# xuhao1/TaichiSLAM

Measured on AMD Instinct MI355X. Metric: depth-frames/s integrated (640x480->512^3 TSDF), higher is better.
Workload: dtype f16 storage / f32 + int64 fixed-point arithmetic; 1 GPU; BASELINE configs[1]: single 640x480 u16 depth stream (sphere room r=3 m, 1 deg/frame) -> DenseTSDF 512^3 / 2 cm, recast_step 2, max_ray 5 m; one stream+submap per GPU

## Files before the change

taichislam_amd/csrc/tsl_integrate.hip:

```cpp
#include "tsl_tsdf.hpp"
#include <hip/hip_ext.h>

namespace tsl {

#ifdef TSL_TIMING
#define TSL_T0() const int _wv = (blockIdx.x * (int)blockDim.x + (int)threadIdx.x) >> 6
#define TSL_TICK(F, k) do { long long _n = wall_clock64(); if (lane_id() == 0 && _wv < 16384) (F).dbg[_wv * 16 + (k)] = _n; } while (0)
#else
#define TSL_T0() do {} while (0)
#define TSL_TICK(F, k) do {} while (0)
#endif

#define SCATTER_TILE 4096

struct RayRegs { float pf0, pf1, pf2, d0, d1, d2, P0, P1, P2, w; long long qden; int n; };

__device__ __forceinline__ uint32_t wave_min_u32(uint32_t v)
{
    for (int d = 32; d > 0; d >>= 1) { const uint32_t o = (uint32_t)__shfl_xor((int)v, d); v = o < v ? o : v; }
    return v;
}
__device__ __forceinline__ RayRegs make_ray(const uint4 rec, int n, const FrameParams& P)
{
    RayRegs R;
// ... 553 lines not shown
{
    if (all_small) {
#pragma unroll
        for (int q = 0; q < N; ++q) nv[q] = apply_update_f(old[q], from_fix32(qn[q]), from_fix32(qd[q]));
    } else {
#pragma unroll
        for (int q = 0; q < N; ++q) nv[q] = apply_update_f(old[q], from_fix(qn[q]), from_fix(qd[q]));
    }
}

__device__ __forceinline__ int uni(int v) { return __builtin_amdgcn_readfirstlane(v); }
#define IT_UNIT 0
#define IT_POOL 1
#define IT_SLAB 2
#define IT_NP   3
#define IT_TMALL 4
#define IT_FMASK 5
#define IT_OFF  6
#define IT_N    (IT_OFF + TSL_NB)
#define IT_WORDS (IT_N + TSL_NB + 2)
#define NRANGE (PLAN_NCLS * (TSL_NB + 1))

template <bool TEX, bool FASTDIV, int NT, int SPT, int WPE>
__global__ void __launch_bounds__(NT, WPE) k_integrate_batch(MapDev M, BatchDev B, int kind)
{
    constexpr int CSEGS = SPT * NT, VPT = TSL_BRK3 / NT, CH = VPT < FLUSH_CHUNK ? VPT : FLUSH_CHUNK;
    static_assert(VPT <= 16, "the written / first-touch masks hold 16 voxels per thread");
#ifdef TSL_EXP_SLOT16
    __shared__ ulonglong2 s_acc[TSL_BRK3];
#define S_NUM(i) s_acc[i].x
#define S_DEN(i) s_acc[i].y
#else
    __shared__ unsigned long long s_num[TSL_BRK3];
    __shared__ unsigned long long s_den[TSL_BRK3];
#define S_NUM(i) s_num[i]
#define S_DEN(i) s_den[i]
#endif
    __shared__ unsigned long long s_keys[CSEGS];
    __shared__ uint32_t s_win[TEX ? TSL_BRK3 : 1];
    __shared__ int s_bin[64];
    __shared__ int s_claim[2];
    __shared__ int s_uq[TSL_NB];
    __shared__ int s_cum[NRANGE + 1];
    __shared__ int s_it[3][IT_WORDS];
    uint32_t okmask = 0u;
#pragma unroll
    for (int q = 0; q < TSL_NB; ++q) if (q < B.n) {
        const FrameDev& Fq = B.f[q];
// ... 51 lines not shown
            int pool = e.z;
            if (fm == 0u) { fm = 1u; pool = -1; }
            it[IT_UNIT] = kq < 0 ? 1 : 0; it[IT_POOL] = pool; it[IT_SLAB] = kq < 0 ? 0 : e.w; it[IT_NP] = kq < 0 ? 1 : (e.y >> 16) & ((1 << PART_NP_BITS) - 1);
            it[IT_TMALL] = (int)tm; it[IT_FMASK] = (int)fm;
        }
    };
    const int r0 = uni(s_claim[0]);
    if (r0 >= total) return;
    { int kq, io, in; const int4 e = entry_of(r0, &kq); info_of(e, kq, &io, &in); commit(0, e, kq, io, in); }
    __syncthreads();
    auto steps_of = [&](int sl, uint32_t fm) -> int {
        int n = 0;
#pragma unroll
        for (int q = 0; q < TSL_NB; ++q) if ((fm >> q) & 1u) n += max(1, (uni(s_it[sl][IT_N + q]) + CSEGS - 1) / CSEGS);
        return n;
    };
    long long uniq = 0;
    int t = 0, slot = 0, c = 0; (void)t;
    int n_known = 0;
    bool exhausted = false;
    int f = __builtin_ctz((uint32_t)uni(s_it[0][IT_FMASK]));

    unsigned long long kk[SPT]; uint4 recs[SPT]; uint32_t wids[SPT];
#define TSL_SORT_DEAL(KIN, NSEG, FD)                                                                                    \
    {                                                                                                                   \
        int rr[SPT];                                                                                                    \
        _Pragma("unroll") for (int q = 0; q < SPT; ++q) {                                                               \
            const int i = q * NT + (int)threadIdx.x; rr[q] = -1;                                                        \
            if (i < (NSEG)) rr[q] = atomicAdd(&s_bin[63 - (int)(KIN[q] & 63ull)], 1);                                   \
        }                                                                                                               \
        __syncthreads();                                                                                                \
        if (threadIdx.x < 64) {                                                                                         \
            const int cb = s_bin[threadIdx.x]; int inc = cb;                                                            \
            for (int d = 1; d < 64; d <<= 1) { const int o = __shfl_up(inc, d); if ((int)threadIdx.x >= d) inc += o; }  \
            s_bin[threadIdx.x] = inc - cb;                                                                              \
        }                                                                                                               \
        __syncthreads();                                                                                                \
        _Pragma("unroll") for (int q = 0; q < SPT; ++q) if (rr[q] >= 0) s_keys[s_bin[63 - (int)(KIN[q] & 63ull)] + rr[q]] = KIN[q]; \
        __syncthreads();                                                                                                \
        _Pragma("unroll") for (int q = 0; q < SPT; ++q) {                                                               \
            const int i = q * NT + ((q & 1) ? NT - 1 - (int)threadIdx.x : (int)threadIdx.x);                            \
            if (i < (NSEG)) {                                                                                           \
                kk[q] = s_keys[i];                                                                                      \
                const int r = (int)((kk[q] >> (SEG_CNT_BITS + SEG_J_BITS)) & ((1u << STG_RAY_BITS) - 1));               \
                recs[q] = (FD).rayA[r];                                                                                 \
                wids[q] = TEX ? (FD).rayFirst[r] + 1u : 0u;                                                             \
            }                                                                                                           \
        }                                                                                                               \
        if (threadIdx.x < 64) s_bin[threadIdx.x] = 0;               \
    }
#define TSL_PRIME(SL, FQ)                                                                                               \
    {                                                                                                                   \
        const FrameDev& F0 = B.f[FQ];                                                                                   \
        const int off0 = uni(s_it[SL][IT_OFF + (FQ)]), nseg0 = min(uni(s_it[SL][IT_N + (FQ)]), CSEGS);                  \
        unsigned long long k0[SPT];                                                                                     \
        _Pragma("unroll") for (int q = 0; q < SPT; ++q) { const int i = q * NT + threadIdx.x; k0[q] = i < nseg0 ? F0.seg_sorted[off0 + i] : 0ull; } \
        TSL_SORT_DEAL(k0, nseg0, F0)                                                                                    \
    }

    {
#ifdef TSL_EXP_SLOT16
        for (int i = threadIdx.x; i < TSL_BRK3; i += NT) s_acc[i] = make_ulonglong2(0ull, 0ull);
#else
        ulonglong2* zn = reinterpret_cast<ulonglong2*>(s_num); ulonglong2* zd = reinterpret_cast<ulonglong2*>(s_den);
        for (int i = threadIdx.x; i < TSL_BRK3 / 2; i += NT) { zn[i] = make_ulonglong2(0ull, 0ull); zd[i] = make_ulonglong2(0ull, 0ull); }
#endif
        if (TEX) for (int i = threadIdx.x; i < TSL_BRK3; i += NT) s_win[i] = 0u;
        if (threadIdx.x < 64) s_bin[threadIdx.x] = 0;
        __syncthreads();
        TSL_PRIME(0, f)
    }
    uint32_t old[VPT];
    uint32_t vmask = 0u;
    bool have_old = false;
    for (;;) {
        const int* const it = s_it[slot];
        const int slot1 = slot == 2 ? 0 : slot + 1, slot2 = slot == 0 ? 2 : slot - 1;
        const bool unit = uni(it[IT_UNIT]) != 0;
        const int p = uni(it[IT_POOL]), rk = uni(it[IT_SLAB]);
        const uint32_t fmask = (uint32_t)uni(it[IT_FMASK]);
        const int n_f = uni(it[IT_N + f]);
        const FrameDev& F = B.f[f];
        const FrameParams& P = *B.p[f];
        const StepK K = { P.vs, P.rvs, P.T[0], P.T[1], P.T[2], M.hN, M.hNz };
        const uint32_t later = fmask >> (f + 1);
        const bool first_frame = (fmask & ((1u << f) - 1u)) == 0u, last_frame = later == 0u;
        const bool first_step = first_frame && c == 0;
        const int nseg = min(CSEGS, n_f - c * CSEGS);
        const bool last_chunk = (c + 1) * CSEGS >= n_f;
        const bool last_step = last_chunk && last_frame;
        int known = max(1, (n_f + CSEGS - 1) / CSEGS) - 1 - c + steps_of(slot, later << (f + 1));
        if (n_known >= 1) known += steps_of(slot1, (uint32_t)uni(s_it[slot1][IT_FMASK]));
        const bool do_claim = !exhausted && n_known < 2 && known <= 1;
        if (do_claim && threadIdx.x == 0) s_claim[0] = __hip_atomic_fetch_add(claim, 1, __ATOMIC_RELAXED, __HIP_MEMORY_SCOPE_AGENT);
#ifdef TSL_TIMING
        long long* const _rec = F.dbg + 131072 + (size_t)blockIdx.x * 128 + (size_t)(t < 16 ? t : 15) * 8;
        if (threadIdx.x == 0 && first_step) { _rec[0] = wall_clock64(); _rec[1] = (unit ? 1 : 0) | (uni(it[IT_NP]) << 8) | ((long long)fmask << 32); _rec[2] = 0; _rec[5] = 0; }
        if (threadIdx.x == 0 && c == 0) _rec[2] += n_f;
        long long* const _ph = F.dbg + 196608 + (size_t)blockIdx.x * 128 + (size_t)(t < 16 ? t : 15) * 8;
        if (threadIdx.x == 0 && first_step) { _ph[0] = _ph[1] = _ph[2] = _ph[3] = _ph[4] = 0; }
        const long long _ta = wall_clock64();
#endif
        const bool has_next = !last_step || n_known >= 1;
        int fx = f, cx = c + 1, slotx = slot;
        if (last_chunk) {
            cx = 0;
            if (!last_frame) fx = f + 1 + __builtin_ctz(later);
            else if (has_next) { slotx = slot1; fx = __builtin_ctz((uint32_t)uni(s_it[slotx][IT_FMASK])); }
        }
        const FrameDev& Fx = B.f[fx];
        unsigned long long kn[SPT];
        const int offx = uni(s_it[slotx][IT_OFF + fx]) + cx * CSEGS;
        const int nsegn = has_next ? min(CSEGS, uni(s_it[slotx][IT_N + fx]) - cx * CSEGS) : 0;
#pragma unroll
        for (int q = 0; q < SPT; ++q) { const int i = q * NT + threadIdx.x; kn[q] = i < nsegn ? Fx.seg_sorted[offx + i] : 0ull; }
        const uint32_t* const twr = M.tw + (size_t)(p >= 0 ? p : 0) * TSL_BRK3;
        if (first_step) { have_old = false; vmask = 0u; }
        if (!TEX && unit && p >= 0 && first_step) {
#pragma unroll
            for (int q = 0; q < VPT; ++q) old[q] = twr[q * NT + threadIdx.x];
            have_old = true;
        }
#pragma unroll
        for (int q = 0; q < SPT; ++q) {
            const int i = q * NT + ((q & 1) ? NT - 1 - (int)threadIdx.x : (int)threadIdx.x);
            if (i >= nseg) continue;
            const unsigned long long key = kk[q];
            const int cnt = (int)(key & ((1u << SEG_CNT_BITS) - 1)), j0 = (int)((key >> SEG_CNT_BITS) & ((1u << SEG_J_BITS) - 1));
            const RayRegs R = make_ray(recs[q], 0, P);
            const uint32_t wid = wids[q];
#ifndef TSL_EXP_STAGGER
#define TSL_EXP_STAGGER 27
#endif
            int off = ((int)((threadIdx.x * (unsigned)TSL_EXP_STAGGER) & 63u) * cnt) >> 6;
            for (int s = 0; s < cnt; s += 2) {
                const int ja = j0 + off; off = (off + 1 == cnt) ? 0 : off + 1;
                const int jb = j0 + off; off = (off + 1 == cnt) ? 0 : off + 1;
                int la, lb; float qa, qb;
                step_eval<FASTDIV>(R, K, ja, &la, &qa);
                step_eval<FASTDIV>(R, K, jb, &lb, &qb);
                long long na = (long long)(int)qa, nb = (long long)(int)qb;
                if (__builtin_expect(__any(!(fabsf(qa) < 2147483648.0f) || !(fabsf(qb) < 2147483648.0f)), 0)) { na = __float2ll_rn(qa); nb = __float2ll_rn(qb); }
                atomicAdd(&S_NUM(la), (unsigned long long)na);
                atomicAdd(&S_DEN(la), (unsigned long long)R.qden);
                if (TEX) atomicMax(&s_win[la], wid);
                const bool vb = s + 1 < cnt;
#ifdef TSL_EXP_ADDZERO
                atomicAdd(&S_NUM(lb), (unsigned long long)(vb ? nb : 0ll));
                atomicAdd(&S_DEN(lb), (unsigned long long)(vb ? R.qden : 0ll));
                if (TEX) atomicMax(&s_win[lb], vb ? wid : 0u);
#else
                if (vb) { atomicAdd(&S_NUM(lb), (unsigned long long)nb); atomicAdd(&S_DEN(lb), (unsigned long long)R.qden); if (TEX) atomicMax(&s_win[lb], wid); }
#endif
            }
        }
        __syncthreads();
#ifdef TSL_TIMING
        if (threadIdx.x == 0 && last_step) _rec[3] = wall_clock64();
        const long long _tb = wall_clock64();
#endif
        bool fetching = false;
        int4 ne = make_int4(0, 0, -1, 0); int nkq = 0, nio = 0, nin = 0;
        if (do_claim) {
            const int r = uni(s_claim[0]);
            if (r < total) { fetching = true; ne = entry_of(r, &nkq); } else exhausted = true;
        }
        if (has_next) TSL_SORT_DEAL(kn, nsegn, Fx)
        if (fetching) info_of(ne, nkq, &nio, &nin);
#ifdef TSL_TIMING
        const long long _tc = wall_clock64();
        if (threadIdx.x == 0) { _ph[0] += _tb - _ta; _ph[1] += _tc - _tb; _ph[4] += 1; }
#endif
        if (!last_chunk) {
            if (fetching) { commit(n_known == 0 ? slot1 : slot2, ne, nkq, nio, nin); ++n_known; __syncthreads(); }
            ++c; continue;
        }
        if (p >= 0 && threadIdx.x == 0) M.touch[p] = 1;
        if (p >= 0 && unit) {
            uint32_t* tw = M.tw + (size_t)p * TSL_BRK3;
            if (!have_old) {
#pragma unroll
                for (int q = 0; q < VPT; ++q) old[q] = tw[q * NT + threadIdx.x];
                have_old = true;
            }
            if (first_frame) {
#pragma unroll
                for (int q = 0; q < VPT; ++q) vmask |= ((old[q] >> 16) == 0u ? 1u : 0u) << (16 + q);
            }
#pragma unroll
            for (int h = 0; h < VPT; h += CH) {
                long long qn[CH], qd[CH]; uint32_t nv[CH]; bool small = true, anyu = false;
#pragma unroll
                for (int q = 0; q < CH; ++q) {
                    const int ls = acc_swz5((h + q) * NT + threadIdx.x);
// ... 35 lines not shown
                S_NUM(ls) = 0ull; S_DEN(ls) = 0ull;
                if (TEX) { F.accw[(size_t)rk * TSL_BRK3 + l] = s_win[ls]; s_win[ls] = 0u; }
            }
        } else {
#ifdef TSL_EXP_SLOT16
            for (int i = threadIdx.x; i < TSL_BRK3; i += NT) s_acc[i] = make_ulonglong2(0ull, 0ull);
#else
            ulonglong2* zn = reinterpret_cast<ulonglong2*>(s_num); ulonglong2* zd = reinterpret_cast<ulonglong2*>(s_den);
            for (int i = threadIdx.x; i < TSL_BRK3 / 2; i += NT) { zn[i] = make_ulonglong2(0ull, 0ull); zd[i] = make_ulonglong2(0ull, 0ull); }
#endif
            if (TEX) for (int i = threadIdx.x; i < TSL_BRK3; i += NT) s_win[i] = 0u;
        }
#ifdef TSL_TIMING
        const long long _td = wall_clock64();
#endif
        {
            const long long u = wave_sum_ll(uniq);
            if (lane_id() == 0 && u) atomicAdd(&s_uq[f], (int)u);
            uniq = 0;
        }
        if (fetching) { commit(n_known == 0 ? slot1 : slot2, ne, nkq, nio, nin); ++n_known; }
#ifdef TSL_TIMING
        if (threadIdx.x == 0 && last_step) _rec[4] = wall_clock64();
        if (threadIdx.x == 0) { _ph[2] += _td - _tc; _ph[3] += wall_clock64() - _td; }
#endif
        if (!has_next && n_known == 0) break;
        __syncthreads();
        c = 0;
        if (last_frame) { ++t; slot = slot1; --n_known; f = __builtin_ctz((uint32_t)uni(s_it[slot][IT_FMASK])); }
        else f = fx;
        if (!has_next) TSL_PRIME(slot, f)
    }
#undef TSL_PRIME
#undef TSL_SORT_DEAL
    __syncthreads();
    if (threadIdx.x < TSL_NB && s_uq[threadIdx.x]) atomic_add_i64(&B.f[threadIdx.x].stats->unique, (long long)s_uq[threadIdx.x]);
}

#ifndef APPLY_SPLIT
#define APPLY_SPLIT 8
#endif
#ifndef APPLY_ROUND
#define APPLY_ROUND 2
#endif
template <bool TEX>
__global__ void __launch_bounds__(256) k_apply_slab(MapDev M, BatchDev B)
{
    __shared__ int s_uq[TSL_NB];
    constexpr int VP = TSL_BRK3 / APPLY_SPLIT / 256;
    uint32_t okmask = 0u;
#pragma unroll
    for (int q = 0; q < TSL_NB; ++q) if (q < B.n && B.f[q].counters[HDR_FAIL] == 0) okmask |= 1u << q;
    const int nheavy = min(B.f[0].counters[HDR_HEAVY], B.f[0].max_frame_bricks);
    const ulonglong2* const slab = reinterpret_cast<const ulonglong2*>(B.f[0].acc);
    if (threadIdx.x < TSL_NB) s_uq[threadIdx.x] = 0;
    __syncthreads();
    for (int item = blockIdx.x; item < nheavy * APPLY_SPLIT; item += gridDim.x) {
        const int4 e = B.f[0].heavy_tab[item / APPLY_SPLIT];
// ... 83 lines not shown

int launch_segments(tsl_tsdf* m, const BatchDev& B, const FrameParams* hp, int total, hipStream_t st)
{
    const FrameParams& P = hp[0];
    if (P.variant != 2) return TSL_OK;
    const int iblocks = (int)(((int64_t)total * P.split + 255) / 256);
    prof_begin(m, TSL_K_SEGMENTS, st);
    if (P.group) hipLaunchKernelGGL(k_segments<true>, dim3(iblocks, B.n), dim3(256), 0, st, m->M, B);
    else hipLaunchKernelGGL(k_segments<false>, dim3(iblocks, B.n), dim3(256), 0, st, m->M, B);
    prof_end(m, st);
    int unit_max = m->unit_max <= m->unit_floor ? m->unit_max : std::max(m->unit_floor, (int)((long long)m->unit_max * B.n / TSL_NB));
    int unit_half = std::min(unit_max, m->unit_half <= 2048 ? m->unit_half : std::max(2048, (int)((long long)m->unit_half * B.n / TSL_NB)));
    if (P.seq && m->seq_impl) unit_max = unit_half = 1 << 30;
    prof_begin(m, TSL_K_BIN, st);
    hipLaunchKernelGGL(k_plan, dim3((B.f[0].max_frame_bricks + 255) / 256, B.n), dim3(256), 0, st, m->M, B, m->chunks * m->wg * m->spt, unit_max, unit_half);
    hipLaunchKernelGGL(k_scatter, dim3(256, B.n), dim3(256), 0, st, B);
    prof_end(m, st);
    return TSL_OK;
}

int launch_brick(tsl_tsdf* m, const BatchDev& B, const FrameParams& P, int kind, hipStream_t st, hipEvent_t start, hipEvent_t stop)
{
    const int bg = kind == 2 ? m->pgrid : (B.n <= 2 ? (m->bgrid + 1) / 2 : (kind == 1 ? m->ugrid : m->bgrid));
#define TSL_LAUNCH_IB(TEXV, FD) do { \
        if (m->wg == 512 && m->spt == 2 && !TEXV) hipExtLaunchKernelGGL((k_integrate_batch<false, FD, 512, 2, 4>), dim3((2 * m->ncu * bg + 99) / 100), dim3(512), 0, st, start, stop, 0, m->M, B, kind); \
        else if (m->wg == 512) hipExtLaunchKernelGGL((k_integrate_batch<TEXV, FD, 512, 4, 2>), dim3((m->ncu * bg + 99) / 100), dim3(512), 0, st, start, stop, 0, m->M, B, kind); \
        else hipExtLaunchKernelGGL((k_integrate_batch<TEXV, FD, 256, 4, (TEXV ? 1 : 2)>), dim3(((TEXV ? 1 : 2) * m->ncu * bg + 99) / 100), dim3(256), 0, st, start, stop, 0, m->M, B, kind); } while (0)
    if (P.tex) { if (P.fastdiv) TSL_LAUNCH_IB(true, true); else TSL_LAUNCH_IB(true, false); }
    else { if (P.fastdiv) TSL_LAUNCH_IB(false, true); else TSL_LAUNCH_IB(false, false); }
#undef TSL_LAUNCH_IB
    TSL_HIP(hipGetLastError());
    return TSL_OK;
}
int launch_slab_apply(tsl_tsdf* m, const BatchDev& B, const FrameParams& P)
{
    prof_begin(m, TSL_K_FINALIZE);
    if (P.tex) hipLaunchKernelGGL(k_apply_slab<true>, dim3(16 * m->ncu), dim3(256), 0, m->stream_, m->M, B);
    else hipLaunchKernelGGL(k_apply_slab<false>, dim3(16 * m->ncu), dim3(256), 0, m->stream_, m->M, B);
    prof_end(m);
    TSL_HIP(hipGetLastError());
    return TSL_OK;
}
int launch_apply_batch(tsl_tsdf* m, const BatchDev& B, const FrameParams& P, hipEvent_t start, hipEvent_t stop)
{
    const int rc = launch_brick(m, B, P, 0, m->stream_, start, stop);
    return rc ? rc : launch_slab_apply(m, B, P);
// ... 20 lines not shown
```

taichislam_amd/csrc/tsl_tsdf.hip:

```cpp
#include "tsl_tsdf.hpp"
#include <rocprim/rocprim.hpp>
#include <algorithm>
#include <cmath>
#include <cstdio>
#include <cstdlib>
#include <cstring>
#include <mutex>

namespace tsl {

static thread_local std::string g_err;
void set_error(const std::string& s) { g_err = s; }

__device__ __forceinline__ uint32_t part1by2_32(uint32_t x)
{
    x &= 0x3ffu;
    x = (x ^ (x << 16)) & 0xff0000ffu;
    x = (x ^ (x << 8)) & 0x0300f00fu;
    x = (x ^ (x << 4)) & 0x030c30c3u;
    x = (x ^ (x << 2)) & 0x09249249u;
    return x;
}
__device__ __forceinline__ uint64_t part1by2_64(uint64_t x)
{
// ... 857 lines not shown
    FrameParams& P = m->P; std::memset(&P, 0, sizeof(P));
    for (int i = 0; i < 3; ++i) P.R[i * 4] = 1.0f;
    P.vs = (float)cfg->voxel_scale;
    {
        const float y0 = (float)(1.0 / (double)P.vs);
        float best = y0; double err = std::fabs(1.0 - (double)y0 * (double)P.vs);
        const float cand[2] = { std::nextafterf(y0, 0.0f), std::nextafterf(y0, INFINITY) };
        for (float c : cand) { const double e = std::fabs(1.0 - (double)c * (double)P.vs); if (e < err) { err = e; best = c; } }
        P.rvs = best; P.fastdiv = 0;
    }
    P.thr_max = (float)(cfg->max_ray_length * 1000.0); P.thr_min = (float)(cfg->min_ray_length * 1000.0);
    P.max_ray_f = (float)cfg->max_ray_length;
    P.max_steps_f = (float)(cfg->max_ray_length / cfg->voxel_scale);
    P.internal_f = (float)cfg->internal_voxels;
    P.pcl_lo = m->pcl_lo; P.pcl_ext = m->pcl_ext; P.pcl_bits = m->pcl_bits; P.pcl_blk = blk; P.seq = 0;
    P.step = cfg->recast_step; P.same_proj = cfg->color_same_proj;
    m->surf_thres = (float)(cfg->voxel_scale * 1.8);
    m->disp_floor = (float)cfg->disp_floor; m->disp_ceiling = (float)cfg->disp_ceiling;
    m->baseR.assign((size_t)m->npose * 9, 0.0); m->baseT.assign((size_t)m->npose * 3, 0.0);
    m->baseRf.assign((size_t)m->npose * 9, 0.0f); m->baseTf.assign((size_t)m->npose * 3, 0.0f);
    for (int s = 0; s < m->npose; ++s) for (int i = 0; i < 3; ++i) { m->baseR[(size_t)s * 9 + i * 4] = 1.0; m->baseRf[(size_t)s * 9 + i * 4] = 1.0f; }
    std::memset(m->gbaseR, 0, sizeof(m->gbaseR)); std::memset(m->gbaseT, 0, sizeof(m->gbaseT));
    for (int i = 0; i < 3; ++i) m->gbaseR[i * 4] = 1.0;
    m->P.group = 1; m->phases = 3; m->wg = 512; m->spt = 2; m->adaptive = 0; m->ramp_batches = 2; m->ramp_size = 4; m->bgrid = 75; m->ugrid = 75; m->pgrid = 25; m->split_launch = 0; m->chunks = 4; m->unit_max = 1024 * TSL_NB; m->unit_half = 1 << 20; m->unit_floor = 4096; m->batch_gen = 0;
    { hipDeviceProp_t pr; TSL_HIP(hipGetDeviceProperties(&pr, device)); m->ncu = pr.multiProcessorCount > 0 ? pr.multiProcessorCount : 256; }
    m->active = 0; m->variant = 2; m->split = 2; m->semantics = 0; m->seq_impl = 1; m->seq_ready = false; m->seq_bytes0 = 0; m->seq_d = nullptr; m->seq_tuple_cap = 0;
    m->prof_on = false; m->prof_open = false; m->prof_group = false; m->prof_mask = ~0u; std::memset(m->prof_ms, 0, sizeof(m->prof_ms)); std::memset(m->prof_n, 0, sizeof(m->prof_n));
    m->sort_temp = nullptr; m->sort_temp_bytes = 0;
    m->xbuf = nullptr; m->xbuf_bytes = 0; m->mesh_v = m->mesh_n = m->mesh_c = nullptr; m->mesh_count = nullptr; m->mesh_cap = 0; m->mesh_flags = nullptr;
    m->fuse_acc = nullptr; m->fuse_cnt = nullptr; m->fuse_cacc = nullptr; m->fuse_dirty = false; m->mrg_nunion = -1;
    m->esdf = nullptr; m->esdf_par = nullptr; m->esdf_ok = nullptr; m->esdf_mode = 0; m->esdf_grid = 0; m->fuse_direct = false; m->merge_exchange = 0; m->mrg_racc = m->mrg_rcnt = m->mrg_rec = nullptr; m->mrg_racc_bytes = m->mrg_rcnt_bytes = m->mrg_rec_bytes = 0; m->esdf_orphans = 0; m->esdf_last = nullptr; m->esdf_in = nullptr; m->esdf_read = nullptr; m->esdf_overlap = true; m->esdf_ctr_idx = 0; for (int k = 0; k < 2; ++k) { m->fseq_keys[k] = m->fseq_vals[k] = nullptr; m->fseq_bytes[k] = m->fseq_vbytes[k] = 0; } m->fseq_temp = nullptr; m->fseq_tbytes = 0; m->fseq_ctr = nullptr; m->esdf_gate = nullptr; m->esdf_gate_ev = nullptr; m->esdf_gate_set = false; m->esdf_gate_mask = 0; m->esdf_valid = false; m->esdf_force_full = false; m->pose_dev = nullptr;

    MapDev& M = m->M; std::memset(&M, 0, sizeof(M));
    M.N = m->N; M.Nz = m->Nz; M.nbx = m->nbx; M.nbz = m->nbz; M.nb3 = m->nb3; M.nsub = m->nsub; M.hN = m->N / 2; M.hNz = m->Nz / 2;
    int64_t want = cfg->max_bricks > 0 ? cfg->max_bricks : 32768 * (int64_t)(m->nsub > 4 ? 4 : (m->nsub > 1 ? m->nsub : 1));
    const int64_t all = (int64_t)m->nsub * m->nb3;
    if (want > all) want = all;
    M.max_bricks = (int)want;
    int rc;
    if ((rc = dev_alloc(m, (void**)&M.table, sizeof(int) * (size_t)all, 0xff))) return rc;
    if ((rc = dev_alloc(m, (void**)&M.tw, sizeof(uint32_t) * (size_t)want * TSL_BRK3, 0))) return rc;
    if ((rc = dev_alloc(m, (void**)&M.obs, (size_t)want * TSL_BRK3, 0))) return rc;
    if ((rc = dev_alloc(m, (void**)&M.occ, (size_t)want * TSL_BRK3, 0))) return rc;
    if (cfg->texture_enabled) { if ((rc = dev_alloc(m, (void**)&M.col, sizeof(uint16_t) * 4 * (size_t)want * TSL_BRK3, 0))) return rc; }
    if ((rc = dev_alloc(m, (void**)&M.owner, sizeof(int) * (size_t)want, 0))) return rc;
    if ((rc = dev_alloc(m, (void**)&M.touch, (size_t)want, 0))) return rc;
    if ((rc = dev_alloc(m, (void**)&M.pool_top, sizeof(int) * 4, 0))) return rc;
// ... 154 lines not shown
    TSL_REQUIRE(m && name && value, "null");
    if (!std::strcmp(name, "group")) { *value = m->P.group; return TSL_OK; }
    if (!std::strcmp(name, "esdf_mode")) { *value = m->esdf_mode; return TSL_OK; }
    if (!std::strcmp(name, "fuse_window_misses")) { return read_int(m, m->M.pool_top + 2, value); }
    if (!std::strcmp(name, "esdf_orphans")) { int rc = esdf_finish(m); if (rc) return rc; *value = (int)m->esdf_orphans; return TSL_OK; }
    if (!std::strcmp(name, "semantics")) { *value = m->semantics; return TSL_OK; }
    if (!std::strcmp(name, "seq_impl")) { *value = m->seq_impl; return TSL_OK; }
    if (!std::strcmp(name, "last_heavy_bricks") || !std::strcmp(name, "last_slab_slots")) {
        TSL_REQUIRE(m->scratch_ready, "nothing integrated yet");
        int rc = tsl_tsdf_sync(m); if (rc) return rc;
        const int bi = (m->cur + TSL_NBATCH - 1) % TSL_NBATCH;
        int v[40];
        TSL_HIP(hipMemcpy(v, m->fset[bi * TSL_NB].F.counters, sizeof(v), hipMemcpyDeviceToHost));
        *value = name[5] == 'h' ? v[14] : v[13];
        return TSL_OK;
    }
    if (!std::strcmp(name, "seq_longest_run")) {
        TSL_REQUIRE(m->scratch_ready, "nothing integrated yet");
        int rc = tsl_tsdf_sync(m); if (rc) return rc;
        const int bi = (m->cur + TSL_NBATCH - 1) % TSL_NBATCH;
        long long sum = 0;
        for (int q = 0; q < m->last_batch_n; ++q) { int v[40]; TSL_HIP(hipMemcpy(v, m->fset[bi * TSL_NB + q].F.counters, sizeof(v), hipMemcpyDeviceToHost)); sum += (unsigned)v[31]; }
        *value = (int)(sum > 0x7fffffffll ? 0x7fffffffll : sum);
        return TSL_OK;
    }
    if (!std::strcmp(name, "seq_long_voxels")) {
        TSL_REQUIRE(m->scratch_ready, "nothing integrated yet");
        int rc = tsl_tsdf_sync(m); if (rc) return rc;
        const int bi = (m->cur + TSL_NBATCH - 1) % TSL_NBATCH;
        int v[40]; TSL_HIP(hipMemcpy(v, m->fset[bi * TSL_NB].F.counters, sizeof(v), hipMemcpyDeviceToHost));
        *value = v[28] + v[30];
#ifdef TSL_SEQ_DBG
        fprintf(stderr, "seq dbg (long role, last batch): evaluations %d, commits that moved T %d, commits that moved W only %d\n", v[32], v[33], v[34]);
#endif
        return TSL_OK;
    }
    if (!std::strcmp(name, "fastdiv")) { *value = m->P.fastdiv; return TSL_OK; }
    if (!std::strcmp(name, "seq_verify_mismatches")) {
        int rc = tsl_tsdf_sync(m); if (rc) return rc;
        std::vector<int> buf(4 + 4 * 64);
        rc = seq_verify_report(m, buf.data(), (int)buf.size()); if (rc) return rc;
        *value = buf[0];
        for (int e = 0; e < buf[0] && e < 64; ++e)
            fprintf(stderr, "seq_verify: batch %d frame %d stage %d slot %d what %d T %d  (stage 3: voxel %d expected %d found %d)\n", buf[4 + 4 * e], buf[5 + 4 * e] & 255, buf[5 + 4 * e] >> 8, buf[6 + 4 * e], buf[7 + 4 * e] & 15, buf[7 + 4 * e] >> 4,
                    buf[7 + 4 * e] & 4095, (buf[7 + 4 * e] >> 12) & 1023, (buf[7 + 4 * e] >> 22) & 1023);
        return TSL_OK;
// ... 379 lines not shown
                return rc;
            }
        }
        return TSL_OK;
    }
    if (!std::strcmp(name, "fastdiv")) { if (value == 0) m->P.fastdiv = 0; return TSL_OK; }
    if (!std::strcmp(name, "mesh_gather")) { m->mesh_gather = value != 0; return TSL_OK; }
    if (!std::strcmp(name, "esdf_full")) { m->esdf_force_full = value != 0; return TSL_OK; }
    if (!std::strcmp(name, "esdf_mode")) { TSL_REQUIRE(value == 0 || value == 1, "esdf_mode: 0 = regional recompute (default), 1 = raise / lower wavefront with parent directions"); int rc = esdf_finish(m); if (rc) return rc; m->esdf_mode = value; m->esdf_valid = false; return TSL_OK; }
    if (!std::strcmp(name, "esdf_round_cap")) { m->esdf_round_cap = value; return TSL_OK; }
    if (!std::strcmp(name, "merge_exchange")) { TSL_REQUIRE(value == 0 || value == 1, "merge_exchange: 0 = all-reduce of the packed sums, 1 = reduce-scatter + all-gather of finalised voxels"); m->merge_exchange = value; return TSL_OK; }
    if (!std::strcmp(name, "fuse_direct")) { m->fuse_direct = value != 0; return TSL_OK; }
    if (!std::strcmp(name, "esdf_grid")) { TSL_REQUIRE(value >= 0, "esdf_grid: workgroups of a relaxation round (0 = four per CU)"); m->esdf_grid = value; return TSL_OK; }
    if (!std::strcmp(name, "esdf_overlap")) { int rc = esdf_finish(m); if (rc) return rc; m->esdf_overlap = value != 0; return TSL_OK; }
    if (!std::strcmp(name, "unit")) { TSL_REQUIRE(value >= 0 && value <= (1 << 20), "unit must be 0..2^20 segments"); int rc = tsl_tsdf_sync(m); if (rc) return rc; m->unit_max = value; return TSL_OK; }
    if (!std::strcmp(name, "unit_floor")) { TSL_REQUIRE(value >= 0 && value <= (1 << 20), "unit_floor must be 0..2^20 segments"); int rc = tsl_tsdf_sync(m); if (rc) return rc; m->unit_floor = value; return TSL_OK; }
    if (!std::strcmp(name, "unit_half")) { TSL_REQUIRE(value >= 0 && value <= (1 << 20), "unit_half must be 0..2^20 segments"); int rc = tsl_tsdf_sync(m); if (rc) return rc; m->unit_half = value; return TSL_OK; }
    if (!std::strcmp(name, "chunks")) { TSL_REQUIRE(value >= 1 && value <= 8, "chunks must be 1..8"); int rc = tsl_tsdf_sync(m); if (rc) return rc; m->chunks = value; return TSL_OK; }
    if (!std::strcmp(name, "adaptive")) { m->adaptive = value != 0; return TSL_OK; }
    if (!std::strcmp(name, "ramp_size")) { TSL_REQUIRE(value >= 1 && value <= TSL_NB, "ramp_size must be 1..8 frames"); m->ramp_size = value; return TSL_OK; }
    if (!std::strcmp(name, "ramp")) { TSL_REQUIRE(value >= 0 && value <= 16, "ramp must be 0..16 half batches"); m->ramp_batches = value; return TSL_OK; }
    if (!std::strcmp(name, "ugrid") || !std::strcmp(name, "pgrid")) { TSL_REQUIRE(value >= 5 && value <= 200, "ugrid / pgrid must be 5..200 (percent of the resident workgroup slots)"); { int rc = tsl_tsdf_sync(m); if (rc) return rc; } (name[0] == 'u' ? m->ugrid : m->pgrid) = value; return TSL_OK; }
    if (!std::strcmp(name, "split_launch")) { TSL_REQUIRE(value == 0 || value == 1, "split_launch must be 0 or 1"); { int rc = tsl_tsdf_sync(m); if (rc) return rc; } m->split_launch = value; return TSL_OK; }
    if (!std::strcmp(name, "bgrid")) { TSL_REQUIRE(value >= 10 && value <= 200, "bgrid must be 10..200 (percent of the resident workgroup slots)"); { int rc = tsl_tsdf_sync(m); if (rc) return rc; } m->bgrid = value; return TSL_OK; }
    if (!std::strcmp(name, "spt")) { TSL_REQUIRE(value == 2 || value == 4, "spt must be 2 or 4"); { int rc = tsl_tsdf_sync(m); if (rc) return rc; } m->spt = value; return TSL_OK; }
    if (!std::strcmp(name, "wg")) { TSL_REQUIRE(value == 256 || value == 512, "wg must be 256 or 512"); { int rc = tsl_tsdf_sync(m); if (rc) return rc; } m->wg = value; return TSL_OK; }
    if (!std::strcmp(name, "phases")) { int rc = tsl_tsdf_sync(m); if (rc) return rc; m->phases = value & 3; return TSL_OK; }
    if (!std::strcmp(name, "overlap")) { int rc = tsl_tsdf_sync(m); if (rc) return rc; m->overlap = value < 0 ? 0 : (value > TSL_NB ? TSL_NB : value); for (auto& H : m->batch) H.b_pending = false; return TSL_OK; }
    if (!std::strcmp(name, "split")) { TSL_REQUIRE(value >= 1 && value <= 64 && (64 % value) == 0, "split must divide 64"); m->split = value; return TSL_OK; }
    set_error("unknown option"); return TSL_ERR_ARG;
}

}
```

taichislam_amd/csrc/tsl_tsdf.hpp:

```cpp
#pragma once
#include "tsl_common.hpp"

namespace tsl {

struct FrameParams {
    float R[9], T[3];
    float fx, fy, cx, cy;
    float fxc, fyc, cxc, cyc;
    float vs;
    float rvs; int fastdiv;
    float thr_max, thr_min;
    float max_ray_f;
    float max_steps_f;
    float internal_f;
    int   pcl_lo, pcl_ext, pcl_bits;
    int   step, hh, ww, H, W;
    int   rstride;
    int   cstride;
    int   th, tw, tex, same_proj;
    int   slot;
    int   variant, split;
    int   group;
    int   seq, pcl_blk;
    int   hlog2;
// ... 35 lines not shown
#define SEG_CNT_BITS 6
#define SEG_J_BITS   12
#define SEG_RAY_BITS 24
#define SEG_SLOT_SHIFT (SEG_CNT_BITS + SEG_J_BITS + SEG_RAY_BITS)
#define SEG_MAX_CNT 63
#define STG_RAY_BITS 22
#define STG_B_SHIFT (SEG_CNT_BITS + SEG_J_BITS + STG_RAY_BITS)
#define PART_NP_BITS 12
#define SLAB_SLOT_BITS 20
#define PLAN_NCLS 4
#define HDR_FAIL 11
#define HDR_CLAIM 12
#define HDR_SLAB 13
#define HDR_HEAVY 14
#define HDR_PARTS 16
#define HDR_UNITS 20
#define HDR_CLAIM2 24
#define HDR_SEQ_TUPLES 26
#define HDR_SEQ_LONG 28
#define HDR_SEQ_XLONG 30
#define HDR_SEQ_MAXRUN 31
#define HDR_SEQ_CLAIM 35
#define HDR_SEQ_SLOTS 29

__device__ __forceinline__ void frame_fail(const MapDev& M, const FrameDev& F, int bits) { atomicOr(&F.counters[11], bits); atomicOr(M.err, bits); }

#define H_INL 13
#define H_BLOCK_SHIFT 44
#define H_EMPTY 0ull
__device__ __forceinline__ unsigned long long h_key(unsigned long long vkey, int block) { return (vkey | ((unsigned long long)block << H_BLOCK_SHIFT)) + 1ull; }
#define GROUP_BIG_CAP 16384
struct HSlot { unsigned long long key; int cnt; uint32_t pix[H_INL]; };
static_assert(sizeof(HSlot) == 64, "one slot per 64 bytes");
__device__ __forceinline__ uint32_t h_hash64(unsigned long long key, int log2n) { return (uint32_t)((key * 0x9E3779B97F4A7C15ull) >> (64 - log2n)); }

struct PixAcc { int cnt; h16 sx, sy, sz, zs, cr, cg, cb; };

__device__ __forceinline__ void acc_colour(const FrameParams& P, const FrameDev& F, uint32_t pid, PixAcc& A)
{
    const uint8_t* rgb;
    if (P.points) rgb = P.tex_input + (size_t)pid * 3;
    else {
        const int jj = (int)pid / P.ww, ii = (int)pid - jj * P.ww;
        const int pj = jj * P.step, pi = ii * P.step;
        if (P.same_proj) rgb = P.tex_input + ((size_t)pj * P.tw + pi) * 3;
        else {
// ... 118 lines not shown
    uint32_t* mesh_flags;
    float *mesh_v, *mesh_n, *mesh_c; int* mesh_count; int64_t mesh_cap; int mesh_gather;
    void *fuse_acc, *fuse_cnt, *fuse_cacc; bool fuse_dirty;
    uint8_t* mrg_mask; int *mrg_list, *mrg_count; int mrg_nunion;
    void *mrg_pacc, *mrg_pcnt; size_t mrg_pacc_bytes, mrg_pcnt_bytes;
    void *mrg_racc, *mrg_rcnt, *mrg_rec; size_t mrg_racc_bytes, mrg_rcnt_bytes, mrg_rec_bytes; int merge_exchange;
    float* esdf; uint8_t *esdf_fl, *esdf_region, *esdf_par, *esdf_ok; int esdf_mode, esdf_grid; bool fuse_direct; long long esdf_orphans; int *esdf_list, *esdf_queue, *esdf_ctr, *esdf_inq, *esdf_nbr; uint32_t* esdf_note; int esdf_qcap;
    float *esdf_exp_xyz, *esdf_exp_val; int* esdf_exp_count; int esdf_exp_n;
    bool esdf_valid, esdf_force_full; int esdf_submap; float esdf_gamma, esdf_maxd; tsl_esdf_stats esdf_stats;
    bool esdf_query_ok; int* esdf_q_ctr; int esdf_q_rounds;
    hipEvent_t esdf_gate, esdf_gate_ev; bool esdf_gate_set; unsigned esdf_gate_mask;
    hipEvent_t esdf_in, esdf_read, esdf_last;
    bool esdf_overlap; int esdf_ctr_idx;
    void *fseq_keys[2], *fseq_vals[2], *fseq_temp; size_t fseq_bytes[2], fseq_vbytes[2], fseq_tbytes; void* fseq_ctr;
    EsdfSlot esdf_slot[TSL_ESDF_SLOTS]; int esdf_tail, esdf_npend, esdf_rounds_seen, esdf_round_cap; bool esdf_short; tsl_esdf_totals_t esdf_tot;
    bool prof_on, prof_open, prof_group; unsigned prof_mask; std::vector<tsl::ProfSlot> prof; std::vector<hipEvent_t> prof_free;
    double prof_ms[TSL_K_COUNT]; int64_t prof_n[TSL_K_COUNT];
    int semantics;
    int seq_impl;
    bool seq_ready; int64_t seq_bytes0;
    tsl::SeqDev seq_h[TSL_NSETS]; tsl::SeqDev* seq_d;
    void *seqb_keys[TSL_NBATCH][2], *seqb_vals[TSL_NBATCH][2], *seqb_temp[TSL_NBATCH], *seqb_long[TSL_NBATCH], *seqb_lmask[TSL_NBATCH], *seqb_perm[TSL_NBATCH]; size_t seqb_temp_bytes; long long seq_tuple_cap;
    unsigned long long *seq_keys[2], *seq_vals[2], *seq_ctr; void* seq_temp; size_t seq_temp_bytes; long long seq_cap;
    int variant, split, phases, wg, spt, ncu, chunks, unit_max, unit_half, unit_floor, bgrid, ugrid, pgrid, split_launch, adaptive, ramp, ramp_batches, ramp_size; bool clean; uint64_t batch_gen;
    int64_t bytes;
    void* seqv_sum[TSL_NBATCH]; int* seqv_log;
    uint32_t shape_hash; int dry_launches;
};

namespace tsl {
int  grow(void** p, size_t* have, size_t need);
hipStream_t ms(tsl_tsdf* m);
int  flush_pending(tsl_tsdf* m);
void prof_begin(tsl_tsdf* m, int kid, hipStream_t st = nullptr, int count = 1);
void prof_end(tsl_tsdf* m, hipStream_t st = nullptr);
bool prof_slot(tsl_tsdf* m, int kid, int count, hipEvent_t* a, hipEvent_t* b);
void convert_pose(const double* Rb, const double* Tb, const double* R, const double* T, float* outR, float* outT);
int  dev_alloc(tsl_tsdf* m, void** p, size_t bytes, int fill);
int  check_variant2(tsl_tsdf* m);
int  launch_segments(tsl_tsdf* m, const BatchDev& B, const FrameParams* hp, int total, hipStream_t st);
int  launch_apply(tsl_tsdf* m, FSet& S, int total);
int  launch_apply_batch(tsl_tsdf* m, const BatchDev& B, const FrameParams& P, hipEvent_t start = nullptr, hipEvent_t stop = nullptr);
int  launch_brick(tsl_tsdf* m, const BatchDev& B, const FrameParams& P, int kind, hipStream_t st, hipEvent_t start, hipEvent_t stop);
int  launch_slab_apply(tsl_tsdf* m, const BatchDev& B, const FrameParams& P);
int  launch_seq_group(tsl_tsdf* m, const BatchDev& B, const FrameParams* hp, int bi, hipStream_t st);
int  launch_seq_apply(tsl_tsdf* m, const BatchDev& B, const FrameParams& P, int bi);
void seq_release(tsl_tsdf* m);
// ... 8 lines not shown
```

Before: 34310 frames/s.

## Split long ray segments across lanes when a brick step has few segments

When a brick step holds at most half a workgroup's worth of segments, each segment is dealt to 2^k lanes, each walking a contiguous sub-range of its voxel steps, with k chosen from the longest segment count (the first key after the sort). The aim is to cut idle lanes and tail latency in sparse bricks, where a handful of long segments had kept most threads idle. It adds a shared-memory read, more divergent setup and extra ray-record loads per split lane. It also adds device counters for split steps, a runtime toggle (on by default) and a timing histogram.

```diff
diff --git a/taichislam_amd/csrc/tsl_integrate.hip b/taichislam_amd/csrc/tsl_integrate.hip
--- a/taichislam_amd/csrc/tsl_integrate.hip
+++ b/taichislam_amd/csrc/tsl_integrate.hip
@@ -599,8 +599,10 @@
 #define NRANGE (PLAN_NCLS * (TSL_NB + 1))
 
 template <bool TEX, bool FASTDIV, int NT, int SPT, int WPE>
-__global__ void __launch_bounds__(NT, WPE) k_integrate_batch(MapDev M, BatchDev B, int kind)
-{
+__global__ void __launch_bounds__(NT, WPE) k_integrate_batch(MapDev M, BatchDev B, int kind_arg)
+{
+    const int kind = kind_arg & 0xff;
+    const bool lsplit = ((kind_arg >> 8) & 1) != 0;
     constexpr int CSEGS = SPT * NT, VPT = TSL_BRK3 / NT, CH = VPT < FLUSH_CHUNK ? VPT : FLUSH_CHUNK;
     static_assert(VPT <= 16, "the written / first-touch masks hold 16 voxels per thread");
 #ifdef TSL_EXP_SLOT16
@@ -698,6 +700,18 @@
     int f = __builtin_ctz((uint32_t)uni(s_it[0][IT_FMASK]));
 
     unsigned long long kk[SPT]; uint4 recs[SPT]; uint32_t wids[SPT];
+    int ksh = 0;
+    int ls_steps = 0, ls_kmask = 0;
+#ifdef TSL_TIMING
+    __shared__ long long s_hist[2][6][4];
+    if (threadIdx.x < 48) (&s_hist[0][0][0])[threadIdx.x] = 0;
+    int mc_dealt = 0;
+#endif
+#ifdef TSL_TIMING
+#define TSL_HIST_MAXCNT(NSEG) mc_dealt = (NSEG) > 0 ? uni((int)(s_keys[0] & ((1u << SEG_CNT_BITS) - 1))) : 0;
+#else
+#define TSL_HIST_MAXCNT(NSEG)
+#endif
 #define TSL_SORT_DEAL(KIN, NSEG, FD)                                                                                    \
     {                                                                                                                   \
         int rr[SPT];                                                                                                    \
@@ -714,13 +728,36 @@
         __syncthreads();                                                                                                \
         _Pragma("unroll") for (int q = 0; q < SPT; ++q) if (rr[q] >= 0) s_keys[s_bin[63 - (int)(KIN[q] & 63ull)] + rr[q]] = KIN[q]; \
         __syncthreads();                                                                                                \
-        _Pragma("unroll") for (int q = 0; q < SPT; ++q) {                                                               \
-            const int i = q * NT + ((q & 1) ? NT - 1 - (int)threadIdx.x : (int)threadIdx.x);                            \
-            if (i < (NSEG)) {                                                                                           \
-                kk[q] = s_keys[i];                                                                                      \
-                const int r = (int)((kk[q] >> (SEG_CNT_BITS + SEG_J_BITS)) & ((1u << STG_RAY_BITS) - 1));               \
-                recs[q] = (FD).rayA[r];                                                                                 \
-                wids[q] = TEX ? (FD).rayFirst[r] + 1u : 0u;                                                             \
+        ksh = 0;                                                                                                        \
+        TSL_HIST_MAXCNT(NSEG)                                                                                           \
+        if (lsplit && (NSEG) > 0 && 2 * (NSEG) <= NT) {                                                                 \
+             \
+            const int maxcnt = uni((int)(s_keys[0] & ((1u << SEG_CNT_BITS) - 1)));                                      \
+            while (ksh < 4 && ((NSEG) << (ksh + 1)) <= NT && maxcnt > (2 << ksh)) ++ksh;                                \
+        }                                                                                                               \
+        if (ksh == 0) {                                                                                                 \
+            _Pragma("unroll") for (int q = 0; q < SPT; ++q) {                                                           \
+                const int i = q * NT + ((q & 1) ? NT - 1 - (int)threadIdx.x : (int)threadIdx.x);                        \
+                if (i < (NSEG)) {                                                                                       \
+                    kk[q] = s_keys[i];                                                                                  \
+                    const int r = (int)((kk[q] >> (SEG_CNT_BITS + SEG_J_BITS)) & ((1u << STG_RAY_BITS) - 1));           \
+                    recs[q] = (FD).rayA[r];                                                                             \
+                    wids[q] = TEX ? (FD).rayFirst[r] + 1u : 0u;                                                         \
+                }                                                                                                       \
+            }                                                                                                           \
+        } else {                                                                                                        \
+             \
+             \
+            ++ls_steps; ls_kmask |= 1 << ksh;                                                                           \
+            const int sg = (int)threadIdx.x >> ksh, sub = (int)threadIdx.x & ((1 << ksh) - 1);                          \
+            if (sg < (NSEG)) {                                                                                          \
+                const unsigned long long key = s_keys[sg];                                                              \
+                const int cnt = (int)(key & ((1u << SEG_CNT_BITS) - 1)), per = (cnt + (1 << ksh) - 1) >> ksh;           \
+                const int mine = min(max(cnt - sub * per, 0), per), skip = mine > 0 ? sub * per : 0;                    \
+                kk[0] = ((key >> SEG_CNT_BITS) + (unsigned long long)skip) << SEG_CNT_BITS | (unsigned long long)mine;  \
+                const int r = (int)((key >> (SEG_CNT_BITS + SEG_J_BITS)) & ((1u << STG_RAY_BITS) - 1));                 \
+                recs[0] = (FD).rayA[r];                                                                                 \
+                wids[0] = TEX ? (FD).rayFirst[r] + 1u : 0u;                                                             \
             }                                                                                                           \
         }                                                                                                               \
         if (threadIdx.x < 64) s_bin[threadIdx.x] = 0;               \
@@ -763,6 +800,7 @@
         const bool first_frame = (fmask & ((1u << f) - 1u)) == 0u, last_frame = later == 0u;
         const bool first_step = first_frame && c == 0;
         const int nseg = min(CSEGS, n_f - c * CSEGS);
+        const int nwalk = nseg << ksh;
         const bool last_chunk = (c + 1) * CSEGS >= n_f;
         const bool last_step = last_chunk && last_frame;
         int known = max(1, (n_f + CSEGS - 1) / CSEGS) - 1 - c + steps_of(slot, later << (f + 1));
@@ -776,6 +814,8 @@
         long long* const _ph = F.dbg + 196608 + (size_t)blockIdx.x * 128 + (size_t)(t < 16 ? t : 15) * 8;
         if (threadIdx.x == 0 && first_step) { _ph[0] = _ph[1] = _ph[2] = _ph[3] = _ph[4] = 0; }
         const long long _ta = wall_clock64();
+        const int _mc = mc_dealt, _band = nseg <= 32 ? 0 : min(5, 27 - __builtin_clz((unsigned)(nseg - 1)));
+        long long* const _h = s_hist[unit ? 1 : 0][_band];
 #endif
         const bool has_next = !last_step || n_known >= 1;
         int fx = f, cx = c + 1, slotx = slot;
@@ -800,7 +840,7 @@
 #pragma unroll
         for (int q = 0; q < SPT; ++q) {
             const int i = q * NT + ((q & 1) ? NT - 1 - (int)threadIdx.x : (int)threadIdx.x);
-            if (i >= nseg) continue;
+            if (i >= nwalk) continue;
             const unsigned long long key = kk[q];
             const int cnt = (int)(key & ((1u << SEG_CNT_BITS) - 1)), j0 = (int)((key >> SEG_CNT_BITS) & ((1u << SEG_J_BITS) - 1));
             const RayRegs R = make_ray(recs[q], 0, P);
@@ -845,7 +885,7 @@
         if (fetching) info_of(ne, nkq, &nio, &nin);
 #ifdef TSL_TIMING
         const long long _tc = wall_clock64();
-        if (threadIdx.x == 0) { _ph[0] += _tb - _ta; _ph[1] += _tc - _tb; _ph[4] += 1; }
+        if (threadIdx.x == 0) { _ph[0] += _tb - _ta; _ph[1] += _tc - _tb; _ph[4] += 1; _h[0] += 1; _h[1] += _tb - _ta; _h[2] += _tc - _tb; _h[3] += _mc; }
 #endif
         if (!last_chunk) {
             if (fetching) { commit(n_known == 0 ? slot1 : slot2, ne, nkq, nio, nin); ++n_known; __syncthreads(); }
@@ -927,7 +967,7 @@
         if (fetching) { commit(n_known == 0 ? slot1 : slot2, ne, nkq, nio, nin); ++n_known; }
 #ifdef TSL_TIMING
         if (threadIdx.x == 0 && last_step) _rec[4] = wall_clock64();
-        if (threadIdx.x == 0) { _ph[2] += _td - _tc; _ph[3] += wall_clock64() - _td; }
+        if (threadIdx.x == 0) { const long long _te = wall_clock64(); _ph[2] += _td - _tc; _ph[3] += _te - _td; _h[2] += _te - _tc; }
 #endif
         if (!has_next && n_known == 0) break;
         __syncthreads();
@@ -938,7 +978,12 @@
     }
 #undef TSL_PRIME
 #undef TSL_SORT_DEAL
+#undef TSL_HIST_MAXCNT
     __syncthreads();
+    if (threadIdx.x == 0 && ls_steps) { atomicAdd(&B.f[0].counters[HDR_LSPLIT_STEPS], ls_steps); atomicOr(&B.f[0].counters[HDR_LSPLIT_KMASK], ls_kmask); }
+#ifdef TSL_TIMING
+    if (threadIdx.x < 48 && gridDim.x <= 448) atomicAdd(reinterpret_cast<unsigned long long*>(B.f[0].dbg + 131072 + 448 * 128 + threadIdx.x), (unsigned long long)(&s_hist[0][0][0])[threadIdx.x]);
+#endif
     if (threadIdx.x < TSL_NB && s_uq[threadIdx.x]) atomic_add_i64(&B.f[threadIdx.x].stats->unique, (long long)s_uq[threadIdx.x]);
 }
 
@@ -1068,6 +1113,7 @@
 int launch_brick(tsl_tsdf* m, const BatchDev& B, const FrameParams& P, int kind, hipStream_t st, hipEvent_t start, hipEvent_t stop)
 {
     const int bg = kind == 2 ? m->pgrid : (B.n <= 2 ? (m->bgrid + 1) / 2 : (kind == 1 ? m->ugrid : m->bgrid));
+    kind |= m->lane_split ? 1 << 8 : 0;
 #define TSL_LAUNCH_IB(TEXV, FD) do { \
         if (m->wg == 512 && m->spt == 2 && !TEXV) hipExtLaunchKernelGGL((k_integrate_batch<false, FD, 512, 2, 4>), dim3((2 * m->ncu * bg + 99) / 100), dim3(512), 0, st, start, stop, 0, m->M, B, kind); \
         else if (m->wg == 512) hipExtLaunchKernelGGL((k_integrate_batch<TEXV, FD, 512, 4, 2>), dim3((m->ncu * bg + 99) / 100), dim3(512), 0, st, start, stop, 0, m->M, B, kind); \
diff --git a/taichislam_amd/csrc/tsl_tsdf.hip b/taichislam_amd/csrc/tsl_tsdf.hip
--- a/taichislam_amd/csrc/tsl_tsdf.hip
+++ b/taichislam_amd/csrc/tsl_tsdf.hip
@@ -903,7 +903,7 @@
     for (int s = 0; s < m->npose; ++s) for (int i = 0; i < 3; ++i) { m->baseR[(size_t)s * 9 + i * 4] = 1.0; m->baseRf[(size_t)s * 9 + i * 4] = 1.0f; }
     std::memset(m->gbaseR, 0, sizeof(m->gbaseR)); std::memset(m->gbaseT, 0, sizeof(m->gbaseT));
     for (int i = 0; i < 3; ++i) m->gbaseR[i * 4] = 1.0;
-    m->P.group = 1; m->phases = 3; m->wg = 512; m->spt = 2; m->adaptive = 0; m->ramp_batches = 2; m->ramp_size = 4; m->bgrid = 75; m->ugrid = 75; m->pgrid = 25; m->split_launch = 0; m->chunks = 4; m->unit_max = 1024 * TSL_NB; m->unit_half = 1 << 20; m->unit_floor = 4096; m->batch_gen = 0;
+    m->P.group = 1; m->phases = 3; m->wg = 512; m->spt = 2; m->adaptive = 0; m->ramp_batches = 2; m->ramp_size = 4; m->bgrid = 75; m->ugrid = 75; m->pgrid = 25; m->split_launch = 0; m->lane_split = 1; m->chunks = 4; m->unit_max = 1024 * TSL_NB; m->unit_half = 1 << 20; m->unit_floor = 4096; m->batch_gen = 0;
     { hipDeviceProp_t pr; TSL_HIP(hipGetDeviceProperties(&pr, device)); m->ncu = pr.multiProcessorCount > 0 ? pr.multiProcessorCount : 256; }
     m->active = 0; m->variant = 2; m->split = 2; m->semantics = 0; m->seq_impl = 1; m->seq_ready = false; m->seq_bytes0 = 0; m->seq_d = nullptr; m->seq_tuple_cap = 0;
     m->prof_on = false; m->prof_open = false; m->prof_group = false; m->prof_mask = ~0u; std::memset(m->prof_ms, 0, sizeof(m->prof_ms)); std::memset(m->prof_n, 0, sizeof(m->prof_n));
@@ -1104,6 +1104,16 @@
         long long sum = 0;
         for (int q = 0; q < m->last_batch_n; ++q) { int v[40]; TSL_HIP(hipMemcpy(v, m->fset[bi * TSL_NB + q].F.counters, sizeof(v), hipMemcpyDeviceToHost)); sum += (unsigned)v[31]; }
         *value = (int)(sum > 0x7fffffffll ? 0x7fffffffll : sum);
+        return TSL_OK;
+    }
+    if (!std::strcmp(name, "lane_split")) { *value = m->lane_split; return TSL_OK; }
+    if (!std::strcmp(name, "lane_split_steps") || !std::strcmp(name, "lane_split_kmask")) {
+        TSL_REQUIRE(m->scratch_ready, "nothing integrated yet");
+        int rc = tsl_tsdf_sync(m); if (rc) return rc;
+        const int bi = (m->cur + TSL_NBATCH - 1) % TSL_NBATCH;
+        int v[40];
+        TSL_HIP(hipMemcpy(v, m->fset[bi * TSL_NB].F.counters, sizeof(v), hipMemcpyDeviceToHost));
+        *value = name[11] == 's' ? v[HDR_LSPLIT_STEPS] : v[HDR_LSPLIT_KMASK];
         return TSL_OK;
     }
     if (!std::strcmp(name, "seq_long_voxels")) {
@@ -1529,6 +1539,7 @@
     if (!std::strcmp(name, "ramp")) { TSL_REQUIRE(value >= 0 && value <= 16, "ramp must be 0..16 half batches"); m->ramp_batches = value; return TSL_OK; }
     if (!std::strcmp(name, "ugrid") || !std::strcmp(name, "pgrid")) { TSL_REQUIRE(value >= 5 && value <= 200, "ugrid / pgrid must be 5..200 (percent of the resident workgroup slots)"); { int rc = tsl_tsdf_sync(m); if (rc) return rc; } (name[0] == 'u' ? m->ugrid : m->pgrid) = value; return TSL_OK; }
     if (!std::strcmp(name, "split_launch")) { TSL_REQUIRE(value == 0 || value == 1, "split_launch must be 0 or 1"); { int rc = tsl_tsdf_sync(m); if (rc) return rc; } m->split_launch = value; return TSL_OK; }
+    if (!std::strcmp(name, "lane_split")) { TSL_REQUIRE(value == 0 || value == 1, "lane_split must be 0 or 1"); { int rc = tsl_tsdf_sync(m); if (rc) return rc; } m->lane_split = value; return TSL_OK; }
     if (!std::strcmp(name, "bgrid")) { TSL_REQUIRE(value >= 10 && value <= 200, "bgrid must be 10..200 (percent of the resident workgroup slots)"); { int rc = tsl_tsdf_sync(m); if (rc) return rc; } m->bgrid = value; return TSL_OK; }
     if (!std::strcmp(name, "spt")) { TSL_REQUIRE(value == 2 || value == 4, "spt must be 2 or 4"); { int rc = tsl_tsdf_sync(m); if (rc) return rc; } m->spt = value; return TSL_OK; }
     if (!std::strcmp(name, "wg")) { TSL_REQUIRE(value == 256 || value == 512, "wg must be 256 or 512"); { int rc = tsl_tsdf_sync(m); if (rc) return rc; } m->wg = value; return TSL_OK; }
diff --git a/taichislam_amd/csrc/tsl_tsdf.hpp b/taichislam_amd/csrc/tsl_tsdf.hpp
--- a/taichislam_amd/csrc/tsl_tsdf.hpp
+++ b/taichislam_amd/csrc/tsl_tsdf.hpp
@@ -81,6 +81,8 @@
 #define HDR_SEQ_MAXRUN 31
 #define HDR_SEQ_CLAIM 35
 #define HDR_SEQ_SLOTS 29
+#define HDR_LSPLIT_STEPS 36
+#define HDR_LSPLIT_KMASK 37
 
 __device__ __forceinline__ void frame_fail(const MapDev& M, const FrameDev& F, int bits) { atomicOr(&F.counters[11], bits); atomicOr(M.err, bits); }
 
@@ -245,7 +247,7 @@
     tsl::SeqDev seq_h[TSL_NSETS]; tsl::SeqDev* seq_d;
     void *seqb_keys[TSL_NBATCH][2], *seqb_vals[TSL_NBATCH][2], *seqb_temp[TSL_NBATCH], *seqb_long[TSL_NBATCH], *seqb_lmask[TSL_NBATCH], *seqb_perm[TSL_NBATCH]; size_t seqb_temp_bytes; long long seq_tuple_cap;
     unsigned long long *seq_keys[2], *seq_vals[2], *seq_ctr; void* seq_temp; size_t seq_temp_bytes; long long seq_cap;
-    int variant, split, phases, wg, spt, ncu, chunks, unit_max, unit_half, unit_floor, bgrid, ugrid, pgrid, split_launch, adaptive, ramp, ramp_batches, ramp_size; bool clean; uint64_t batch_gen;
+    int variant, split, phases, wg, spt, ncu, chunks, unit_max, unit_half, unit_floor, bgrid, ugrid, pgrid, split_launch, lane_split, adaptive, ramp, ramp_batches, ramp_size; bool clean; uint64_t batch_gen;
     int64_t bytes;
     void* seqv_sum[TSL_NBATCH]; int* seqv_log;
     uint32_t shape_hash; int dry_launches;
```

Measured after the change: 34350 frames/s (median of 4 runs). No clear change (+0.1%).
